# wingolab-org/pecaller

Measured on AMD Instinct MI355X. Metric: M reads mapped/sec (whole node), 2x150bp PE synthetic hg38, higher is better.
Workload: dtype f64

## Files before the change

### include/pemap_hip.h

```cpp
#ifndef PEMAP_HIP_H
#define PEMAP_HIP_H
#include <stdint.h>
#include <stddef.h>

#ifdef __cplusplus
extern "C" {
#endif

#define PEMAP_MAX_HITS   200
#define PEMAP_MIN_READ   16
#define PEMAP_MAX_READ   278

enum
{
  PEMAP_UNIQUE_MATE = 0, PEMAP_UNIQUE_SLIP = 1, PEMAP_UNIQUE_SINGLE = 2, PEMAP_UNIQUE_MIS = 3, PEMAP_NON_MATE = 4,
  PEMAP_NON_MIS = 5, PEMAP_FRAG_MIS = 6, PEMAP_NON_NO = 7, PEMAP_NEITHER_MAP = 8
};

typedef struct pemap_dev pemap_dev;

typedef void (*pemap_ins_cb) (void *user, uint32_t pos, const char *seq, int len);

const char *pemap_dev_last_error (const pemap_dev * dev);

// ... 50 lines not shown
int pemap_dev_staged_reads (pemap_dev * dev, char *reads1, int *len1, char *reads2, int *len2, int stride);
int pemap_dev_staged_info (pemap_dev * dev, int *n, int *stride, int *paired);
int pemap_dev_free (pemap_dev * dev, void *d_ptr);

typedef struct
{
  int32_t n, got[2], end[2], bad_len[2];
  uint64_t consumed[2];
} pemap_fastq_result;
int pemap_dev_stage_fastq (pemap_dev * dev, const char *text1, uint64_t bytes1, int state1, const char *text2, uint64_t bytes2, int state2,
                           int trim_start, int trim_end, int max_records, int stride, pemap_fastq_result * res);
int pemap_dev_submit_fastq (pemap_dev * dev, const char *text1, uint64_t bytes1, int state1, const char *text2, uint64_t bytes2, int state2,
                            int trim_start, int trim_end, int max_records, int stride, uint32_t * m1, uint32_t * m2, int *mapping_type,
                            pemap_fastq_result * res, uint64_t * ticket);

int pemap_dev_fetch_pileup (pemap_dev * dev, uint16_t * counts, pemap_ins_cb cb, void *user);
int pemap_dev_fetch_records (pemap_dev * dev, uint64_t first, uint64_t count, void *out, uint64_t out_capacity,
                             uint64_t * n_records);
int pemap_dev_reset_pileup (pemap_dev * dev);
int pemap_dev_absorb (pemap_dev * dst, pemap_dev * src);

int pemap_dev_summary (pemap_dev * dev, long *out13);

int pemap_dev_run_stats (pemap_dev * dev, uint64_t * stats17, float *times_ms8);

int pemap_dev_debug_hits (pemap_dev * dev, int *n_hits, uint32_t * spot, uint8_t * orient, uint32_t * win_start,
                          int *win_len, double *score, int *start_k, int *start_i);

typedef struct pecall_dev pecall_dev;
int pecall_dev_create (pecall_dev ** out, int device_id);
void pecall_dev_destroy (pecall_dev * dev);
const char *pecall_dev_last_error (const pecall_dev * dev);
int pecall_dev_site_like (pecall_dev * dev, const uint16_t * reads, const double *alpha_mean, int n_sites, int indiv,
                          int max_gen, int min_depth, double norm, double *like, int8_t * best, double *margin);
int pecall_dev_stage (pecall_dev * dev, const uint16_t * reads, const double *alpha_mean, int n_sites, int indiv);
int pecall_dev_run (pecall_dev * dev, int n_sites, int indiv, int max_gen, int min_depth, double norm, int sync);
int pecall_dev_collect (pecall_dev * dev, int n_sites, int indiv, double *like, int8_t * best, double *margin);

int pecall_dev_call_sites (pecall_dev * dev, const uint16_t * reads, const uint8_t * ref_base, const uint8_t * chrom_type, long n_sites,
                           int indiv, int haploid, double threshold, double theta, int8_t * call, double *posterior,
                           int8_t * site_type, int32_t * allele_count, int8_t * n_pass, int32_t * denovo);
int pecall_dev_call_sites_sparse (pecall_dev * dev, const uint16_t * reads, const uint8_t * ref_base, const uint8_t * chrom_type, long n_sites,
                                  int indiv, int haploid, double threshold, double theta, int8_t * call, uint32_t * post_site,
                                  double *post_rows, uint64_t post_cap, uint64_t * n_post, int8_t * site_type, int32_t * allele_count,
                                  int8_t * n_pass, int32_t * denovo);
int pecall_dev_pin_host (pecall_dev * dev, const void *host_ptr, uint64_t n_bytes);
int pecall_dev_unpin_host (pecall_dev * dev, const void *host_ptr);
// ... 39 lines not shown
```

### pecaller_amd/csrc/pemap_capi.hip

```cpp
#include <stdio.h>
#include <stdlib.h>
#include <string.h>
#include <stdarg.h>
#include <unistd.h>
#include <cstring>
#include <memory>
#include <mutex>
#include <thread>
#include <type_traits>
#include <vector>
#include "../../include/pemap_hip.h"
#include "pemap_kernels.hip.h"
#include "pemap_aux.hip.h"
#include "pemap_fastq.hip.h"
#include <rocprim/rocprim.hpp>

static char g_create_err[512] = "";
struct PmChunkCtr;

#define PM_RING 3
struct PmRingSlot
{
  bool active = false;
  unsigned long long seq = 0;
// ... 41 lines not shown
{
  char *base;
  size_t bytes;
  int users;
};
static std::mutex g_pin_mu;
static std::vector < PmPinned > g_pinned;


struct PmKnobs
{
  int big_blocks_per_cu, sw_waves_per_cu;
  int replicas;
  int gapless;
  double dir_budget_gb;
  int lookup_waves ;
  int lookup_prio, vote_prio, sw_prio;
  int vote_waves;
  int walk_blocks_per_cu, pile_blocks_per_cu;
  int pipeline;
  int chunk_pairs;
  int gapless_blocks_per_cu;
  int band, band_waves_per_cu;
  int first_tier;
  int tier2_waves;
  int absorb_staged;
  size_t absorb_chunk;
};

static int env_int (const char *name, int dflt)
{
  const char *e = getenv (name);
  return (e && *e) ? atoi (e) : dflt;
}

static void read_knobs (PmKnobs & k)
{
  k.big_blocks_per_cu = env_int ("PEMAP_BIG_BLOCKS_PER_CU", 8);
  k.sw_waves_per_cu = env_int ("PEMAP_SW_WAVES_PER_CU", 16);
  if (k.big_blocks_per_cu < 1) k.big_blocks_per_cu = 1;
  if (k.sw_waves_per_cu < 1) k.sw_waves_per_cu = 1;
  k.replicas = getenv ("PEMAP_REPLICAS") ? (env_int ("PEMAP_REPLICAS", 1) ? 1 : 0) : -1;
  k.gapless = env_int ("PEMAP_GAPLESS", 3);
  { const char *e = getenv ("PEMAP_DIR_BUDGET_GB"); k.dir_budget_gb = e ? atof (e) : 40.0; if (k.dir_budget_gb < 0.25) k.dir_budget_gb = 0.25; }
  k.lookup_waves = env_int ("PEMAP_LOOKUP_WAVES", -1);
  k.lookup_prio = env_int ("PEMAP_LOOKUP_PRIO", 0);
  k.tier2_waves = env_int ("PEMAP_TIER2_WAVES", 3);
  if (k.tier2_waves < 1) k.tier2_waves = 1;
  k.first_tier = env_int ("PEMAP_FIRST_TIER", 1);
  k.vote_prio = env_int ("PEMAP_VOTE_PRIO", 0);
  k.sw_prio = env_int ("PEMAP_SW_PRIO", 0);
  k.vote_waves = env_int ("PEMAP_VOTE_WAVES", 1024);
  if (k.vote_waves < 1) k.vote_waves = 1;
  k.walk_blocks_per_cu = env_int ("PEMAP_WALK_BLOCKS_PER_CU", 4);
  k.pile_blocks_per_cu = env_int ("PEMAP_PILE_BLOCKS_PER_CU", 4);
  if (k.walk_blocks_per_cu < 1) k.walk_blocks_per_cu = 1;
  if (k.pile_blocks_per_cu < 1) k.pile_blocks_per_cu = 1;
  k.pipeline = env_int ("PEMAP_PIPELINE", 1);
  k.chunk_pairs = env_int ("PEMAP_CHUNK_PAIRS", 262144);
  k.band = env_int ("PEMAP_BAND", 1);
  k.gapless_blocks_per_cu = env_int ("PEMAP_GAPLESS_BLOCKS_PER_CU", -1);
  if (k.gapless_blocks_per_cu == 0) k.gapless_blocks_per_cu = 1;
  k.band_waves_per_cu = env_int ("PEMAP_BAND_WAVES_PER_CU", 16);
  if (k.band_waves_per_cu < 1) k.band_waves_per_cu = 1;
  k.absorb_staged = env_int ("PEMAP_ABSORB_STAGED", 0) ? 1 : 0;
  const int kib = env_int ("PEMAP_ABSORB_CHUNK", 262144);
  k.absorb_chunk = kib > 0 ? ((size_t) kib * 1024) & ~(size_t) 255 : 0;
  if (k.absorb_chunk < 256) k.absorb_chunk = 256;
}

struct PmFastqMate
{
  uint8_t *d_text = nullptr;
  size_t text_cap = 0;
  unsigned *d_tile_cnt = nullptr;
  size_t tile_cap = 0;
  unsigned *d_line_start = nullptr;
  size_t line_cap = 0;
  PfqTileSum *d_sums = nullptr;
  uint2 *d_tile_in = nullptr;
  size_t ltile_cap = 0;
  unsigned *d_rec_off = nullptr, *d_rec_next = nullptr;
  int *d_rec_len = nullptr;
// ... 449 lines not shown
      HIPCHK (d, hipDeviceSynchronize ());
      return build_replicas (d);
    }
  return 0;
}

extern "C" int pemap_dev_lookup_replicas (pemap_dev * d, int *n_replicas, uint64_t * record_bytes)
{
  *n_replicas = d->n_rep;
  if (record_bytes)
    *record_bytes = d->n_rep ? d->multi_units * 16ull : 0ull;
  return 0;
}

extern "C" int pemap_dev_seed_launch (pemap_dev * d, int *asked, int *resident, int *launched, int *lds_bytes)
{
  *asked = d->seed_launch[0];
  *resident = d->seed_launch[1];
  *launched = d->seed_launch[2];
  *lds_bytes = d->seed_launch[3];
  return 0;
}

extern "C" int pemap_dev_index_commit (pemap_dev * d)
{
  if (!d->d_pos_index)
    return fail (d, "index_commit: no index arrays allocated");
  HIPCHK (d, hipSetDevice (d->device));
  HIPCHK (d, hipDeviceSynchronize ());
  TRY (build_replicas (d));
  d->index_ready = true;
  return 0;
}

extern "C" int pemap_dev_load_index (pemap_dev * d, const uint32_t * pos_index, const uint32_t * mers, uint64_t n_mers,
                                     const char *genome, uint64_t genome_size, const uint32_t * contig_starts, int n_contigs,
                                     int idepth)
{
  TRY (pemap_dev_index_alloc (d, n_mers, genome_size, n_contigs, idepth));
  HIPCHK (d, hipMemcpy (d->d_pos_index, pos_index, POS_INDEX_N * sizeof (uint32_t), hipMemcpyHostToDevice));
  HIPCHK (d, hipMemcpy (d->d_mers, mers, n_mers * sizeof (uint32_t), hipMemcpyHostToDevice));
  HIPCHK (d, hipMemcpy (d->d_genome, genome, genome_size, hipMemcpyHostToDevice));
  HIPCHK (d, hipMemcpy (d->d_contig_starts, contig_starts, ((size_t) n_contigs + 1) * sizeof (uint32_t), hipMemcpyHostToDevice));
  return pemap_dev_index_commit (d);
}

// ... 275 lines not shown
{
  int lanes, w;
  pick_geom (d, L, &lanes, &w);
  return (L + 21 + lanes + 15) & ~15;
}

static size_t slab_dwords_for (const pemap_dev * d, int L)
{
  int lanes, W;
  pick_geom (d, L, &lanes, &W);
  return (size_t) lanes * (size_t) tstride_for (d, L) * (size_t) ((W * 4 + 31) / 32);
}

static size_t dir_budget_bytes (const pemap_dev * d)
{
  return (size_t) (d->kn.dir_budget_gb * 1073741824.0);
}

#define PM_TASK_QUARTERS 4
struct PmTaskList
{
  uint32_t *all, *dp, *band, *c3;
  unsigned *n_all, *n_dp, *n_band, *n_c3, *dp_next, *band_next;
};

static size_t task_quarter_words (int n_ends, bool multi)
{
  return (size_t) n_ends * (multi ? PM_MAX_HITS : 1);
}

static PmTaskList task_list (const pemap_dev * d, const PmChunkSet & S, PmCounters * ctr, bool multi)
{
  uint32_t *const t = multi ? S.tasks_m : S.tasks_s;
  const size_t q = task_quarter_words (d->cap_ends, multi);
  const bool rule = pm_gapless_on (d);
  PmTaskList l;
  l.all = t;
  l.n_all = multi ? &ctr->n_tasks_m : &ctr->n_tasks_s;
  l.dp = rule ? t + q : l.all;
  l.n_dp = !rule ? l.n_all : multi ? &ctr->n_tasks_mdp : &ctr->n_tasks_dp;
  l.band = rule && d->kn.band ? t + 2 * q : nullptr;
  l.c3 = rule && pm_gapless_max_x (d) >= 3 ? t + 3 * q : nullptr;
  l.n_band = &ctr->n_band[multi];
  l.n_c3 = &ctr->n_c3[multi];
  l.dp_next = &ctr->sw_next[multi];
  l.band_next = &ctr->band_next[multi];
  return l;
}

static int alloc_hits (pemap_dev * d, PmHits & h, int n_ends)
{
  size_t nh = (size_t) n_ends * PM_MAX_HITS;
  TRY (dev_alloc (d, &h.n_hits, (size_t) n_ends));
  TRY (dev_alloc (d, &h.slot, (size_t) n_ends));
  TRY (dev_alloc (d, &h.spot, nh));
  TRY (dev_alloc (d, &h.gpos, nh));
  TRY (dev_alloc (d, &h.nn, nh));
  TRY (dev_alloc (d, &h.orient, nh));
  TRY (dev_alloc (d, &h.score, nh));
  TRY (dev_alloc (d, &h.sti, nh));
  TRY (dev_alloc (d, &h.stk, nh));
  return 0;
}

static int ensure_work (pemap_dev * d, int n_ends)
// ... 296 lines not shown
    HIPCHK (d, hipStreamWaitEvent (s.seed, *copy_ev, 0));
  if (g >= PM_SETS)
    HIPCHK (d, hipStreamWaitEvent (s.seed, S.ev_lists_free, 0));
  if (pm_fused (d))
    {
      if (g >= PM_SETS && s.ahead)
        HIPCHK (d, hipStreamWaitEvent (s.seed, S.ev_walk_done, 0));
      launch_lookup (d, c, S, cc, ev, s.seed);
      launch_rest (d, c, S, cc, s.seed);
      if (!s.emit_on_alu)
        launch_emit (d, c, S, cc, ev, s.seed);
    }
  else
    launch_lookup (d, c, S, cc, ev, s.seed);
  HIPCHK (d, hipEventRecord (S.ev_lists_ready, s.seed));
  return 0;
}

template < bool C3 > static void launch_gapless (pemap_dev * d, bool short_rows, int ggrid, const RunCtx & c, const PmChunkSet & S, const uint32_t * tasks,
                                                 const unsigned *n_tasks, const PmTaskList & l, int max_x, uint32_t * tasks_c3, unsigned *n_tasks_c3)
{
  if (short_rows)
    hipLaunchKernelGGL (HIP_KERNEL_NAME (pm_gapless_kernel < C3, true >), dim3 (ggrid), dim3 (PM_GL_BLOCK), 0, d->stream, c.ix, c.b, c.prm, S.hits, tasks, n_tasks,
                        l.dp, l.n_dp, max_x, l.band, l.n_band, tasks_c3, n_tasks_c3);
  else
    hipLaunchKernelGGL (HIP_KERNEL_NAME (pm_gapless_kernel < C3, false >), dim3 (ggrid), dim3 (PM_GL_BLOCK), 0, d->stream, c.ix, c.b, c.prm, S.hits, tasks, n_tasks,
                        l.dp, l.n_dp, max_x, l.band, l.n_band, tasks_c3, n_tasks_c3);
}

template < int W, int LPA, bool DIRS > static auto launch_cascade (pemap_dev * d, const RunCtx & c, const PmChunkSet & S, PmCounters * ctr, const PmTaskList & l)
{
  const int n_ends = c.b.n_ends, max_x = pm_gapless_max_x (d);
  int ggrid = d->n_cus * 16, bgrid = d->n_cus * d->kn.band_waves_per_cu;
  if (DIRS)
    {
      const int gbp = d->kn.gapless_blocks_per_cu > 0 ? d->kn.gapless_blocks_per_cu : (seg_template (c.L) <= 10 ? 24 : 4);
      ggrid = (n_ends + PM_GL_PER_BLOCK - 1) / PM_GL_PER_BLOCK;
      if (ggrid > d->n_cus * gbp)
        ggrid = d->n_cus * gbp;
      if (bgrid > (n_ends + 15) / 16)
        bgrid = (n_ends + 15) / 16;
    }
  const bool short_rows = seg_template (c.L) <= 10;
  if (pm_gapless_on (d))
    launch_gapless < false > (d, short_rows, ggrid, c, S, l.all, l.n_all, l, max_x, l.c3, l.n_c3);
  if (l.c3)
    launch_gapless < true > (d, short_rows, ggrid, c, S, l.c3, l.n_c3, l, max_x, (uint32_t *) nullptr, (unsigned *) nullptr);
  if (l.band)
    hipLaunchKernelGGL (HIP_KERNEL_NAME (pm_band_kernel < DIRS >), dim3 (bgrid), dim3 (64), 0, d->stream, c.ix, c.b, c.prm, S.hits, l.band, l.n_band, ctr,
                        S.dirbuf, slab_dwords_for (d, c.L), l.band_next);
  hipLaunchKernelGGL (HIP_KERNEL_NAME (pm_sw_kernel < W, LPA, DIRS >), dim3 (d->sw_grid), dim3 (64), 0, d->stream, c.ix, c.b, c.prm, S.hits, l.dp, l.n_dp, ctr,
                      S.dirbuf, S.dirbuf + c.dump_off, c.tstride, c.L, d->kn.sw_prio, l.dp_next);
}

template < int W, int LPA > static void launch_chunk (pemap_dev * d, const PmSchedule & s, const RunCtx & c, uint32_t * m1, uint32_t * m2, int *mt,
                                             PmChunkSet & S, PmChunkCtr * cc, hipEvent_t * ev)
{
  const PmHits & H = S.hits;
  uint32_t *wins = S.wins, *dirbuf = S.dirbuf;
  PmCounters *ctr = &cc->c;
  if (!pm_fused (d))
    {
      launch_vote (d, c, S, cc, ev, d->stream);
      launch_rest (d, c, S, cc, d->stream);
      launch_emit (d, c, S, cc, ev, d->stream);
    }
  else if (s.emit_on_alu)
    launch_emit (d, c, S, cc, ev, d->stream);
  launch_cascade < W, LPA, true > (d, c, S, ctr, task_list (d, S, ctr, false));
  hipEventRecord (ev[PM_EV_SW_SINGLE_END], d->stream);
// ... 40 lines not shown
            fprintf (stderr, "[pm_s4_probe]");
            for (int i = 0; i < 16; i++)
              fprintf (stderr, " %s %.1f%%", nm[i], 100.0 * (double) pr[i] / (double) tot);
            fprintf (stderr, " | total %.3f G wave-cycles | segments %llu, dropped for a too-many bucket %llu, of them by the k-mer's own bucket %llu\n", (double) tot / 1e9, pr[16], pr[17], pr[18]);
            fprintf (stderr, "[pm_s4_probe] ends decoded %llu; passed over: the list's room %llu, positions next to candidates %llu\n", pr[20], pr[21], pr[23]);
          }
        (void) hipMemcpyToSymbol (HIP_SYMBOL (pm_s4_probe), z, sizeof z);
      }
  }
#endif
  std::vector < PmChunkCtr > hc (nch);
  HIPCHK (d, hipMemcpy (hc.data (), d->d_chunk_ctr, sizeof (PmChunkCtr) * nch, hipMemcpyDeviceToHost));
  HIPCHK (d, hipMemcpy (&d->last_cur, d->d_cur, sizeof (PmInsCursor), hipMemcpyDeviceToHost));
  PmCounters & t = d->last_ctr;
  for (int k = 0; k < nch; k++)
    {
      const PmCounters & c = hc[k].c;
      t.n_tasks_s += c.n_tasks_s;
      t.n_tasks_m += c.n_tasks_m;
      t.n_tasks_dp += pm_gapless_on (d) ? c.n_tasks_dp : c.n_tasks_s;
      t.n_tasks_mdp += pm_gapless_on (d) ? c.n_tasks_mdp : c.n_tasks_m;
      t.n_band[0] += c.n_band[0];
      t.n_band[1] += c.n_band[1];
      t.cells_band += c.cells_band;
      t.n_slots += c.n_slots;
      t.n_redo += c.n_redo;
      t.n_wins += c.n_wins;
      t.n_walks += c.n_walks;
      t.positions += c.positions + hc[k].positions;
      t.cells_score += c.cells_score;
      t.cells_dirs += c.cells_dirs;
      t.pile_incs += c.pile_incs;
      t.n_ins += c.n_ins;
      d->last_big += hc[k].n_big;
      d->last_big2 += hc[k].n_big2;
      hipEvent_t *ev = &d->evs[(size_t) k * PM_NEV];
      float ms = 0.f;
      for (const auto & iv : pm_intervals)
        if (hipEventElapsedTime (&ms, ev[iv.from], ev[iv.to]) == hipSuccess)
          {
            d->last_ms[iv.slot] += ms;
            d->last_ms[PM_T_SEED] += iv.seed_too ? ms : 0.f;
          }
    }
  if (d->last_cur.ins_overflow)
    return fail (d, "insertion log overflow (%u bytes): lower PEMAP_CHUNK_PAIRS or map smaller slices", d->ins_cap);
// ... 619 lines not shown
extern "C" int pemap_dev_run_stats (pemap_dev * d, uint64_t * s, float *t)
{
  TRY (pemap_dev_sync (d));
  const PmCounters & c = d->last_ctr;
  if (s)
    {
      s[0] = d->run_ends;
      s[1] = c.positions;
      s[2] = (uint64_t) c.n_tasks_s + c.n_tasks_m;
      s[3] = (uint64_t) c.n_tasks_dp + c.n_band[0] + c.n_redo;
      s[4] = c.cells_score;
      s[5] = c.cells_dirs;
      s[6] = c.pile_incs;
      s[7] = c.n_ins;
      s[8] = c.n_wins;
      s[9] = c.n_redo;
      s[10] = d->last_big;
      s[11] = (uint64_t) d->run_chunks;
      s[12] = ((uint64_t) c.n_tasks_s - c.n_tasks_dp - c.n_band[0]) + ((uint64_t) c.n_tasks_m - c.n_tasks_mdp - c.n_band[1]);
      s[13] = (uint64_t) c.n_band[0] + c.n_band[1];
      s[14] = c.cells_band;
      s[15] = d->last_big2;
      s[16] = c.n_walks;
    }
  if (t)
    memcpy (t, d->last_ms, sizeof (d->last_ms));
  return 0;
}

extern "C" int pemap_dev_debug_hits (pemap_dev * d, int *n_hits, uint32_t * spot, uint8_t * orient, uint32_t * win_start,
                                     int *win_len, double *score, int *start_k, int *start_i)
{
  HIPCHK (d, hipSetDevice (d->device));
  HIPCHK (d, hipStreamSynchronize (d->stream));
  const int n_ends = d->paired ? 2 * d->run_n : d->run_n;
  const size_t nh = (size_t) n_ends * PM_MAX_HITS;
  const PmHits & H = d->set[0].hits;
  if (n_hits)
    HIPCHK (d, hipMemcpy (n_hits, H.n_hits, (size_t) n_ends * sizeof (int), hipMemcpyDeviceToHost));
  if (spot)
    HIPCHK (d, hipMemcpy (spot, H.spot, nh * 4, hipMemcpyDeviceToHost));
  if (orient)
    HIPCHK (d, hipMemcpy (orient, H.orient, nh, hipMemcpyDeviceToHost));
  if (win_start)
    HIPCHK (d, hipMemcpy (win_start, H.gpos, nh * 4, hipMemcpyDeviceToHost));
  if (score)
// ... 609 lines not shown
```

### pecaller_amd/csrc/pemap_kernels.hip.h

```cpp
#pragma once
#include <hip/hip_runtime.h>
#include <stdint.h>
#include "pemap_pile_diff.h"

#define PM_MAX_HITS 200
#define PM_TOO_MANY 100
#define PM_SLOP 10
#define PM_MAX_SEG 19
#define PM_SEED_CAP 1024
#define PM_SEG_LIST_MAX 4851
#define PM_WAVES_PER_EU(W) ((W) <= 13 ? 4 : (W) <= 19 ? 3 : (W) <= 32 ? 2 : 1)
#define PM_SW_WAVES_PER_EU(W, DIRS) ((W) <= 10 ? 4 : (W) <= 13 ? 3 : (W) <= 16 ? ((DIRS) ? 3 : 2) : ((DIRS) ? 2 : 3))

struct PmIndex
{
  const uint32_t *pos_index;
  const uint32_t *mers;
  const uint8_t *genome;
  const uint32_t *contig_starts;
  uint64_t n_mers;
  uint64_t gsize;
  int n_contigs;
  int idepth;
  const uint32_t *rep;
// ... 59 lines not shown
  return (uint16_t) (p.w[(size_t) q * p.plane_words + (pos >> 1)] >> (16 * (pos & 1)));
}

struct PmCounters
{
  unsigned int n_tasks_s;
  unsigned int n_tasks_m;
  unsigned int n_slots;
  unsigned int n_redo;
  unsigned int n_wins;
  unsigned int n_tasks_dp;
  unsigned long long positions;
  unsigned long long cells_score;
  unsigned long long cells_dirs;
  unsigned long long pile_incs;
  unsigned long long n_ins;
  unsigned int sw_next[3];
  unsigned int n_tasks_mdp;
  unsigned int n_band[2];
  unsigned int band_next[2];
  unsigned int n_c3[2];
  unsigned long long cells_band;
  unsigned int n_walks;
};

struct PmInsCursor
{
  unsigned int ins_bytes;
  unsigned int ins_overflow;
};

struct PmHits
{
  int *n_hits;
  uint32_t *spot;
  uint32_t *gpos;
  int16_t *nn;
  uint8_t *orient;
  double *score;
  int16_t *sti;
  uint8_t *stk;
  int *slot;
};

struct PmBatch
{
// ... 123 lines not shown
```

### pecaller_amd/csrc/pemap_sw.hip.h

```cpp
#pragma once

#define PM_GO 2.0
#define PM_GE (1.0 / 36.0)
#define PM_NEGBIG (-1.0e30)

__device__ __forceinline__ double pm_border (int j)
{
  return -(PM_GO + (double) (j - 1) * PM_GE);
}

__device__ __forceinline__ double pm_top (int j)
{
  return (j >= 1) ? pm_border (j) : (double) j;
}

__device__ __forceinline__ double pm_max (double a, double b)
{
  return __builtin_fmax (a, b);
}

__device__ __forceinline__ bool pm_match (uint8_t r, uint8_t q, int bis)
{
  bool m = (r == q) | (q == 'N') | (q == 'n');
  m |= (r == 'N') & (q >= 'N');
// ... 341 lines not shown
{
  const uint64_t vv = v | (0x4141414141414141ull & ~(~0ull << vacated_bits));
  const uint32_t lo = (uint32_t) vv, hi = (uint32_t) (vv >> 32);
  const uint32_t clo = pm_comp4 (lo), chi = pm_comp4 (hi);
  if (pm_comp4 (clo) == lo && pm_comp4 (chi) == hi)
    return ((uint64_t) __builtin_amdgcn_perm (0u, clo, 0x00010203u) << 32) | (uint64_t) __builtin_amdgcn_perm (0u, chi, 0x00010203u);
  uint64_t w = 0;
#pragma unroll
  for (int k = 0; k < 8; k++)
    w |= (uint64_t) pm_rc_flat ((uint8_t) (v >> (8 * (7 - k)))) << (8 * k);
  return w;
}

#define PM_GAPLESS 4
#define PM_GL_QUEUE 32
#define PM_GL_QUEUE_SHORT 24

#ifndef PM_BAND_K
#define PM_BAND_K 5
#endif
#define PM_BAND_W (22 + 2 * PM_BAND_K)
#define PM_BAND_MAXX_ (PM_BAND_K >= 5 ? 6 : PM_BAND_K + 1)
static_assert (PM_BAND_K >= 2 && PM_BAND_K <= 5, "the band holds at most 32 diagonals");
#define PM_GL_BLOCK 64
#define PM_GL_PER_BLOCK (PM_GL_BLOCK / 32)
#ifndef PM_GL_WAVES_PER_EU
#define PM_GL_WAVES_PER_EU 4
#endif
#define PM_GL_SHORT_MM 160
template < bool SHORT > struct PmGlRows
{
  static constexpr int RD = SHORT ? (PM_GL_SHORT_MM + 7) / 8 * 8 : 320;
  static constexpr int WIN = SHORT ? 16 + (PM_GL_SHORT_MM + 2 * PM_SLOP + 1 + 15) / 8 * 8 : 360;
  static constexpr int QUEUE = SHORT ? PM_GL_QUEUE_SHORT : PM_GL_QUEUE;
};
static_assert (PmGlRows < true >::RD == 160 && PmGlRows < true >::WIN == 208, "short rows as derived above");
static_assert (PM_GL_PER_BLOCK * (PmGlRows < true >::RD + PmGlRows < true >::WIN) + 3 * 4 * PmGlRows < true >::QUEUE <= 1024, "the short form's LDS budget");
template < bool C3, bool SHORT > __global__ __launch_bounds__ (PM_GL_BLOCK, PM_GL_WAVES_PER_EU) void pm_gapless_kernel (PmIndex ix, PmBatch b, PmParams prm, PmHits h, const uint32_t * tasks,
                                                          const unsigned *n_tasks_p, uint32_t * tasks_dp, unsigned *n_tasks_dp, int max_x,
                                                          uint32_t * tasks_band, unsigned *n_tasks_band, uint32_t * tasks_c3, unsigned *n_tasks_c3)
{
  using Rows = PmGlRows < SHORT >;
  constexpr int QN = Rows::QUEUE;
  __shared__ __align__ (8) uint8_t rd[PM_GL_PER_BLOCK][Rows::RD];
  __shared__ __align__ (8) uint8_t win[PM_GL_PER_BLOCK][Rows::WIN];
  __shared__ uint32_t q_band[PM_GL_BLOCK / 64][QN], q_dp[PM_GL_BLOCK / 64][QN];
  __shared__ uint32_t q_c3[PM_GL_BLOCK / 64][C3 ? 1 : QN];
  const int wv = threadIdx.x >> 6;
  int n_qb = 0, n_qd = 0, n_q3 = 0;
  auto flush_queue = [&] (const uint32_t * q, int &n, uint32_t * dst, unsigned *counter)
  {
    if (n == 0)
      return;
    const unsigned base = (unsigned) __builtin_amdgcn_readfirstlane ((int) ((threadIdx.x & 63) == 0 ? atomicAdd (counter, (unsigned) n) : 0u));
    __builtin_amdgcn_fence (__ATOMIC_SEQ_CST, "wavefront");
    __builtin_amdgcn_wave_barrier ();
    if ((int) (threadIdx.x & 63) < n)
      dst[base + (threadIdx.x & 63)] = q[threadIdx.x & 63];
    n = 0;
    __builtin_amdgcn_fence (__ATOMIC_SEQ_CST, "wavefront");
    __builtin_amdgcn_wave_barrier ();
  };
  const int lane = threadIdx.x & 63, l = lane & 31, half = lane & 32;
  const int slot = threadIdx.x >> 5;
  const unsigned n_tasks = *n_tasks_p;
  const int bis = prm.bisulfite;
  const double miss = __hiloint2double ((int) 0xBFD55555u, (int) 0x55555555u);
  const unsigned stride = gridDim.x * (unsigned) PM_GL_PER_BLOCK;
  struct Meta
  {
    size_t o;
    int mm, nn, orient;
// ... 304 lines not shown
      double sc = 0.0;
      if ((cmask >> l) & 1u)
        {
          if (mism >= 1)
            {
              sc = (double) m1 + miss;
              int at = m1;
              for (int k = 1; k < mism; k++)
                {
                  const int nxt = k == 1 ? m2 : mlast;
                  sc = pm_add_ones (sc, nxt - at - 1);
                  sc = sc + miss;
                  at = nxt;
                }
              sc = pm_add_ones (sc, mm - at - 1);
            }
          else
            sc = (double) mm;
        }
      {
        int xmin = mism;
        for (int s = 16; s; s >>= 1)
          xmin = min (xmin, __shfl_xor (xmin, s));
        const bool to_c3 = !C3 && valid && cmask == 0u && l == 0 && tasks_c3 && xmin == 3 && ndiag == 2 * PM_SLOP + 2;
        const bool open = valid && cmask == 0u && l == 0 && !to_c3;
        const bool to_band = open && tasks_band && xmin <= PM_BAND_MAXX_, to_dp = open && !to_band;
        const unsigned long long mb = __ballot (to_band), md = __ballot (to_dp);
        if (to_band)
          q_band[wv][n_qb + (int) __popcll (mb & ((1ull << lane) - 1ull))] = (uint32_t) o;
        if (to_dp)
          q_dp[wv][n_qd + (int) __popcll (md & ((1ull << lane) - 1ull))] = (uint32_t) o;
        n_qb += (int) __popcll (mb);
        n_qd += (int) __popcll (md);
        if (n_qb > QN - 2)
          flush_queue (q_band[wv], n_qb, tasks_band, n_tasks_band);
        if (n_qd > QN - 2)
          flush_queue (q_dp[wv], n_qd, tasks_dp, n_tasks_dp);
        if (!C3)
          {
            const unsigned long long m3 = __ballot (to_c3);
            if (to_c3)
              q_c3[wv][n_q3 + (int) __popcll (m3 & ((1ull << lane) - 1ull))] = (uint32_t) o;
            n_q3 += (int) __popcll (m3);
            if (n_q3 > QN - 2)
              flush_queue (q_c3[wv], n_q3, tasks_c3, n_tasks_c3);
          }
      }
      if (valid)
        {
// ... 8 lines not shown
                  m &= m - 1u;
                  const double s = __shfl (sc, half + dl);
                  if (bd < 0 || s > best)
                    {
                      best = s;
                      bd = dl;
                    }
                }
              if (l == 0)
                {
                  h.score[o] = best;
                  h.stk[o] = (uint8_t) PM_GAPLESS;
                  h.sti[o] = (int16_t) (bd + mm);
                }
            }
        }
      __builtin_amdgcn_fence (__ATOMIC_SEQ_CST, "wavefront");
      __builtin_amdgcn_wave_barrier ();
    }
  flush_queue (q_band[wv], n_qb, tasks_band, n_tasks_band);
  flush_queue (q_dp[wv], n_qd, tasks_dp, n_tasks_dp);
  if (!C3)
    flush_queue (q_c3[wv], n_q3, tasks_c3, n_tasks_c3);
}

__device__ __forceinline__ int pm_wave_max (int v)
{
  for (int o = 32; o > 0; o >>= 1)
    v = max (v, __shfl_xor (v, o));
  return v;
}

template < int W, int PM_LPA, bool DIRS > __global__ __launch_bounds__ (64, PM_SW_WAVES_PER_EU (W, DIRS)) void pm_sw_kernel (PmIndex ix, PmBatch b, PmParams prm, PmHits h,
                                                                                              const uint32_t * tasks,
                                                                                              const unsigned *n_tasks_p, PmCounters * ctr,
                                                                                              uint32_t * dirbuf, uint32_t * dump_slab, int tstride,
                                                                                              int mm_fill, int prio, unsigned *next_task)
{
  constexpr int TPW = 64 / PM_LPA;
  __shared__ uint32_t stage[DIRS ? 64 * PM_STAGE_OF (PmSwGeom < W >::DW) * PmSwGeom < W >::DW : 4];
  __shared__ uint32_t *slab_of_group[TPW + 1];
  pm_set_prio (prio);
  const int lane = threadIdx.x;
  const int q = lane / PM_LPA;
  const unsigned n_tasks = *n_tasks_p;
  if (blockIdx.x * (unsigned) TPW >= n_tasks)
// ... 564 lines not shown
```

### pecaller_amd/pemap.py

```python
import ctypes as C
import os
import numpy as np

HERE = os.path.dirname(os.path.abspath(__file__))
LIB_PATH = os.environ.get("PEMAP_LIB") or os.path.join(HERE, "libpemap_hip.so")
MAX_HITS = 200
MIN_READ = 16
MAX_READ = 278
CLASS_NAMES = ["UNIQUE_MATE", "UNIQUE_SLIP", "UNIQUE_SINGLE", "UNIQUE_MIS", "NON_MATE", "NON_MIS", "FRAG_MIS", "NON_NO",
               "NEITHER_MAP"]

SYMBOLS = [
    "pemap_dev_last_error", "pemap_dev_create", "pemap_dev_destroy", "pemap_dev_load_index", "pemap_dev_build_index",
    "pemap_dev_build_index_resident", "pemap_dev_index_alloc", "pemap_dev_index_commit", "pemap_dev_set_lookup_replicas",
    "pemap_dev_lookup_replicas", "pemap_dev_buffer",
    "pemap_dev_index_info", "pemap_dev_read_buffer", "pemap_dev_set_params", "pemap_dev_map_batch",
    "pemap_dev_submit_batch", "pemap_dev_wait_batch", "pemap_dev_pin_host", "pemap_dev_unpin_host",
    "pemap_dev_stage_reads", "pemap_dev_run", "pemap_dev_run_slice", "pemap_dev_collect", "pemap_dev_sync",
    "pemap_dev_synth_genome", "pemap_dev_synth_reads", "pemap_dev_synth_reads_indel", "pemap_dev_staged_reads", "pemap_dev_staged_info",
    "pemap_dev_free", "pemap_dev_fetch_pileup", "pemap_dev_fetch_records", "pemap_dev_reset_pileup", "pemap_dev_summary",
    "pemap_dev_run_stats", "pemap_dev_debug_hits", "pemap_dev_index_share", "pemap_dev_absorb",
    "pecall_dev_create", "pecall_dev_destroy", "pecall_dev_last_error", "pecall_dev_site_like", "pecall_dev_stage",
    "pecall_dev_run", "pecall_dev_collect", "pecall_dev_call_sites", "pecall_dev_call_sites_sparse", "pecall_dev_set_pedigree",
    "pecall_dev_sites_stage", "pecall_dev_sites_run", "pecall_dev_sites_stats", "pecall_dev_sites_collect", "pecall_dev_pin_host", "pecall_dev_unpin_host",
    "pecall_dev_sites_stage_records", "pecall_dev_sites_gather", "pecall_dev_sites_merge_ms", "pecall_dev_call_records",
    "pecall_dev_sites_stage_records_guided", "pecall_dev_call_records_guided",
    "pecall_dev_sites_base_text",
    "pemap_dev_stage_fastq", "pemap_dev_submit_fastq", "pemap_dev_seed_launch",
]

FASTQ_TILE = 4096
FASTQ_LINE_TILE = 1024
FASTQ_TOP = 1024
FASTQ_MAX_TEXT = 1 << 30


class FastqResult(C.Structure):
    _fields_ = [("n", C.c_int32), ("got", C.c_int32 * 2), ("end", C.c_int32 * 2), ("bad_len", C.c_int32 * 2), ("consumed", C.c_uint64 * 2)]

    def as_dict(self):
        return dict(n=self.n, got=list(self.got), end=list(self.end), bad_len=list(self.bad_len), consumed=list(self.consumed))


PILE_DT = np.dtype([("pos", "<u4"), ("c", "<u2", (6,))])
# ... 32 lines not shown
        L.pemap_dev_read_buffer.argtypes = [vp, i, u64, vp, u64]
        L.pemap_dev_set_params.argtypes = [vp, i, i, i, dbl, i]
        L.pemap_dev_map_batch.argtypes = [vp, vp, vp, vp, vp, i, i, vp, vp, vp]
        L.pemap_dev_submit_batch.argtypes = [vp, vp, vp, vp, vp, i, i, vp, vp, vp, C.POINTER(u64)]
        L.pemap_dev_wait_batch.argtypes = [vp, u64]
        L.pemap_dev_pin_host.argtypes = [vp, vp, u64]
        L.pemap_dev_unpin_host.argtypes = [vp, vp]
        L.pemap_dev_stage_reads.argtypes = [vp, vp, vp, vp, vp, i, i]
        L.pemap_dev_run.argtypes = [vp, i]
        L.pemap_dev_run_slice.argtypes = [vp, i, i, i]
        L.pemap_dev_collect.argtypes = [vp, vp, vp, vp]
        L.pemap_dev_sync.argtypes = [vp]
        L.pemap_dev_synth_genome.argtypes = [vp, u64, u64, i, dbl, C.POINTER(vp), vp]
        L.pemap_dev_synth_reads.argtypes = [vp, u64, i, i, i, dbl, dbl, u64]
        L.pemap_dev_synth_reads_indel.argtypes = [vp, u64, i, i, i, dbl, dbl, u64]
        L.pemap_dev_staged_reads.argtypes = [vp, vp, vp, vp, vp, i]
        L.pemap_dev_staged_info.argtypes = [vp, C.POINTER(i), C.POINTER(i), C.POINTER(i)]
        L.pemap_dev_free.argtypes = [vp, vp]
        L.pemap_dev_fetch_pileup.argtypes = [vp, vp, vp, vp]
        L.pemap_dev_fetch_records.argtypes = [vp, u64, u64, vp, u64, C.POINTER(u64)]
        L.pemap_dev_reset_pileup.argtypes = [vp]
        L.pemap_dev_summary.argtypes = [vp, vp]
        L.pemap_dev_run_stats.argtypes = [vp, vp, vp]
        L.pemap_dev_debug_hits.argtypes = [vp, vp, vp, vp, vp, vp, vp, vp, vp]
        L.pemap_dev_index_share.argtypes = [vp, vp]
        L.pemap_dev_absorb.argtypes = [vp, vp]
        fq = [vp, C.c_char_p, u64, i, C.c_char_p, u64, i, i, i, i, i]
        L.pemap_dev_stage_fastq.argtypes = fq + [C.POINTER(FastqResult)]
        L.pemap_dev_submit_fastq.argtypes = fq + [vp, vp, vp, C.POINTER(FastqResult), C.POINTER(u64)]
        _lib = L
    return _lib


INS_CB = C.CFUNCTYPE(None, C.c_void_p, C.c_uint32, C.c_char_p, C.c_int)


def _p(a):
    return None if a is None else a.ctypes.data


class PemapDev:

    def __init__(self, device_id=0):
        self.L = load_library()
        h = C.c_void_p()
        if self.L.pemap_dev_create(C.byref(h), device_id):
# ... 35 lines not shown
        self._ck(self.L.pemap_dev_index_alloc(self.h, n_mers, genome_size, n_contigs, idepth))
        self.gsize = genome_size

    def index_commit(self):
        self._ck(self.L.pemap_dev_index_commit(self.h))

    def index_share(self, src):
        self._ck(self.L.pemap_dev_index_share(self.h, src.h))
        self.gsize = src.gsize

    def set_lookup_replicas(self, n):
        self._ck(self.L.pemap_dev_set_lookup_replicas(self.h, int(n)))

    def lookup_replicas(self):
        n = C.c_int(0)
        b = C.c_uint64(0)
        self._ck(self.L.pemap_dev_lookup_replicas(self.h, C.byref(n), C.byref(b)))
        return n.value, b.value

    def seed_launch(self):
        v = [C.c_int(0) for _ in range(4)]
        self._ck(self.L.pemap_dev_seed_launch(self.h, *[C.byref(x) for x in v]))
        return dict(zip(("asked", "resident", "launched", "lds_bytes"), (x.value for x in v)))

    def index_info(self):
        a, b, c, d = C.c_uint64(), C.c_uint64(), C.c_int(), C.c_int()
        self._ck(self.L.pemap_dev_index_info(self.h, C.byref(a), C.byref(b), C.byref(c), C.byref(d)))
        return a.value, b.value, c.value, d.value

    def buffer(self, which):
        p, n = C.c_void_p(), C.c_uint64()
        self._ck(self.L.pemap_dev_buffer(self.h, which, C.byref(p), C.byref(n)))
        return p.value, n.value

    def read_buffer(self, which, dtype, offset_bytes=0, n_bytes=None):
        _, nb = self.buffer(which)
        if n_bytes is None:
            n_bytes = nb - offset_bytes
        out = np.empty(n_bytes // np.dtype(dtype).itemsize, dtype=dtype)
        self._ck(self.L.pemap_dev_read_buffer(self.h, which, offset_bytes, _p(out), n_bytes))
        return out

    def set_params(self, paired=True, min_dist=0, max_dist=500, min_align=0.85, bisulfite=False):
        self.paired = bool(paired)
        self._ck(self.L.pemap_dev_set_params(self.h, int(paired), min_dist, max_dist, min_align, int(bisulfite)))

# ... 120 lines not shown
        return counts, sorted(ins)

    def fetch_records(self, first=0, count=None):
        count = self.gsize - first if count is None else count
        n = C.c_uint64()
        self._ck(self.L.pemap_dev_fetch_records(self.h, first, count, None, 0, C.byref(n)))
        out = np.zeros(n.value, PILE_DT)
        if n.value:
            self._ck(self.L.pemap_dev_fetch_records(self.h, first, count, _p(out), n.value, C.byref(n)))
        return out

    def reset_pileup(self):
        self._ck(self.L.pemap_dev_reset_pileup(self.h))

    def absorb(self, src):
        self._ck(self.L.pemap_dev_absorb(self.h, src.h))

    def summary(self):
        out = np.zeros(13, np.int64)
        self._ck(self.L.pemap_dev_summary(self.h, _p(out)))
        return out

    def run_stats(self):
        s = np.zeros(17, np.uint64)
        t = np.zeros(8, np.float32)
        self._ck(self.L.pemap_dev_run_stats(self.h, _p(s), _p(t)))
        keys = ["ends", "positions", "sw_score", "sw_dirs", "cells_score", "cells_dirs", "pile_incs", "n_ins", "walks", "redo", "big_ends", "chunks", "gapless", "banded", "cells_band", "mono_ends", "walked"]
        tk = ["seed", "sw_single", "sw_multi", "select", "sw_redo", "walk", "lookup", "vote"]
        return dict(zip(keys, (int(x) for x in s))), dict(zip(tk, (float(x) for x in t)))

    def debug_hits(self, n_ends):
        nh = np.zeros(n_ends, np.int32)
        spot = np.zeros((n_ends, MAX_HITS), np.uint32)
        orient = np.zeros((n_ends, MAX_HITS), np.uint8)
        ws = np.zeros((n_ends, MAX_HITS), np.uint32)
        wl = np.zeros((n_ends, MAX_HITS), np.int32)
        sc = np.zeros((n_ends, MAX_HITS), np.float64)
        sk = np.zeros((n_ends, MAX_HITS), np.int32)
        si = np.zeros((n_ends, MAX_HITS), np.int32)
        self._ck(self.L.pemap_dev_debug_hits(self.h, _p(nh), _p(spot), _p(orient), _p(ws), _p(wl), _p(sc), _p(sk), _p(si)))
        return dict(n_hits=nh, spot=spot, orient=orient, win_start=ws, win_len=wl, score=sc, start_k=sk, start_i=si)
```

Measured before the change: 118.3.

## Gate high-mismatch gapless candidates into the banded kernel instead of full DP

Ends that fail the gapless mismatch threshold and span two or more diagonals are now sent to the C3 gapless pass. There, a wave-level bound built from the first and last mismatch positions decides whether a small-band indel alignment could reach the best score. Ends that pass this gate go to the banded kernel rather than full Smith-Waterman DP, to cut expensive DP work. This adds a routing pass, shuffles and an atomic counter. By default it is disabled for small batches relative to the SW grid.

```diff
diff --git a/include/pemap_hip.h b/include/pemap_hip.h
--- a/include/pemap_hip.h
+++ b/include/pemap_hip.h
@@ -96,7 +96,9 @@
 
 int pemap_dev_summary (pemap_dev * dev, long *out13);
 
-int pemap_dev_run_stats (pemap_dev * dev, uint64_t * stats17, float *times_ms8);
+int pemap_dev_sw_grid (pemap_dev * dev);
+
+int pemap_dev_run_stats (pemap_dev * dev, uint64_t * stats18, float *times_ms8);
 
 int pemap_dev_debug_hits (pemap_dev * dev, int *n_hits, uint32_t * spot, uint8_t * orient, uint32_t * win_start,
                           int *win_len, double *score, int *start_k, int *start_i);
diff --git a/pecaller_amd/csrc/pemap_capi.hip b/pecaller_amd/csrc/pemap_capi.hip
--- a/pecaller_amd/csrc/pemap_capi.hip
+++ b/pecaller_amd/csrc/pemap_capi.hip
@@ -87,6 +87,7 @@
   int chunk_pairs;
   int gapless_blocks_per_cu;
   int band, band_waves_per_cu;
+  int band_gate;
   int first_tier;
   int tier2_waves;
   int absorb_staged;
@@ -124,6 +125,7 @@
   k.pipeline = env_int ("PEMAP_PIPELINE", 1);
   k.chunk_pairs = env_int ("PEMAP_CHUNK_PAIRS", 262144);
   k.band = env_int ("PEMAP_BAND", 1);
+  k.band_gate = getenv ("PEMAP_BAND_GATE") ? (env_int ("PEMAP_BAND_GATE", 1) ? 1 : 0) : -1;
   k.gapless_blocks_per_cu = env_int ("PEMAP_GAPLESS_BLOCKS_PER_CU", -1);
   if (k.gapless_blocks_per_cu == 0) k.gapless_blocks_per_cu = 1;
   k.band_waves_per_cu = env_int ("PEMAP_BAND_WAVES_PER_CU", 16);
@@ -619,6 +621,11 @@
   return 0;
 }
 
+extern "C" int pemap_dev_sw_grid (pemap_dev * d)
+{
+  return d->sw_grid;
+}
+
 extern "C" int pemap_dev_index_commit (pemap_dev * d)
 {
   if (!d->d_pos_index)
@@ -940,6 +947,7 @@
 {
   uint32_t *all, *dp, *band, *c3;
   unsigned *n_all, *n_dp, *n_band, *n_c3, *dp_next, *band_next;
+  unsigned *n_gate;
 };
 
 static size_t task_quarter_words (int n_ends, bool multi)
@@ -958,7 +966,8 @@
   l.dp = rule ? t + q : l.all;
   l.n_dp = !rule ? l.n_all : multi ? &ctr->n_tasks_mdp : &ctr->n_tasks_dp;
   l.band = rule && d->kn.band ? t + 2 * q : nullptr;
-  l.c3 = rule && pm_gapless_max_x (d) >= 3 ? t + 3 * q : nullptr;
+  l.n_gate = l.band && d->kn.band_gate ? &ctr->n_gate[multi] : nullptr;
+  l.c3 = rule && (pm_gapless_max_x (d) >= 3 || l.n_gate) ? t + 3 * q : nullptr;
   l.n_band = &ctr->n_band[multi];
   l.n_c3 = &ctr->n_c3[multi];
   l.dp_next = &ctr->sw_next[multi];
@@ -1301,15 +1310,18 @@
 {
   if (short_rows)
     hipLaunchKernelGGL (HIP_KERNEL_NAME (pm_gapless_kernel < C3, true >), dim3 (ggrid), dim3 (PM_GL_BLOCK), 0, d->stream, c.ix, c.b, c.prm, S.hits, tasks, n_tasks,
-                        l.dp, l.n_dp, max_x, l.band, l.n_band, tasks_c3, n_tasks_c3);
+                        l.dp, l.n_dp, max_x, l.band, l.n_band, tasks_c3, n_tasks_c3, l.n_gate);
   else
     hipLaunchKernelGGL (HIP_KERNEL_NAME (pm_gapless_kernel < C3, false >), dim3 (ggrid), dim3 (PM_GL_BLOCK), 0, d->stream, c.ix, c.b, c.prm, S.hits, tasks, n_tasks,
-                        l.dp, l.n_dp, max_x, l.band, l.n_band, tasks_c3, n_tasks_c3);
+                        l.dp, l.n_dp, max_x, l.band, l.n_band, tasks_c3, n_tasks_c3, l.n_gate);
 }
 
 template < int W, int LPA, bool DIRS > static auto launch_cascade (pemap_dev * d, const RunCtx & c, const PmChunkSet & S, PmCounters * ctr, const PmTaskList & l)
 {
   const int n_ends = c.b.n_ends, max_x = pm_gapless_max_x (d);
+  PmTaskList lg = l;
+  if (d->kn.band_gate < 0 && (long) n_ends <= (long) d->sw_grid * (64 / LPA))
+    lg.n_gate = nullptr;
   int ggrid = d->n_cus * 16, bgrid = d->n_cus * d->kn.band_waves_per_cu;
   if (DIRS)
     {
@@ -1322,9 +1334,9 @@
     }
   const bool short_rows = seg_template (c.L) <= 10;
   if (pm_gapless_on (d))
-    launch_gapless < false > (d, short_rows, ggrid, c, S, l.all, l.n_all, l, max_x, l.c3, l.n_c3);
+    launch_gapless < false > (d, short_rows, ggrid, c, S, l.all, l.n_all, lg, max_x, l.c3, l.n_c3);
   if (l.c3)
-    launch_gapless < true > (d, short_rows, ggrid, c, S, l.c3, l.n_c3, l, max_x, (uint32_t *) nullptr, (unsigned *) nullptr);
+    launch_gapless < true > (d, short_rows, ggrid, c, S, l.c3, l.n_c3, lg, max_x, (uint32_t *) nullptr, (unsigned *) nullptr);
   if (l.band)
     hipLaunchKernelGGL (HIP_KERNEL_NAME (pm_band_kernel < DIRS >), dim3 (bgrid), dim3 (64), 0, d->stream, c.ix, c.b, c.prm, S.hits, l.band, l.n_band, ctr,
                         S.dirbuf, slab_dwords_for (d, c.L), l.band_next);
@@ -1411,6 +1423,8 @@
       t.n_tasks_mdp += pm_gapless_on (d) ? c.n_tasks_mdp : c.n_tasks_m;
       t.n_band[0] += c.n_band[0];
       t.n_band[1] += c.n_band[1];
+      t.n_gate[0] += c.n_gate[0];
+      t.n_gate[1] += c.n_gate[1];
       t.cells_band += c.cells_band;
       t.n_slots += c.n_slots;
       t.n_redo += c.n_redo;
@@ -2076,6 +2090,7 @@
       s[14] = c.cells_band;
       s[15] = d->last_big2;
       s[16] = c.n_walks;
+      s[17] = (uint64_t) c.n_gate[0] + c.n_gate[1];
     }
   if (t)
     memcpy (t, d->last_ms, sizeof (d->last_ms));
diff --git a/pecaller_amd/csrc/pemap_kernels.hip.h b/pecaller_amd/csrc/pemap_kernels.hip.h
--- a/pecaller_amd/csrc/pemap_kernels.hip.h
+++ b/pecaller_amd/csrc/pemap_kernels.hip.h
@@ -105,6 +105,7 @@
   unsigned int n_c3[2];
   unsigned long long cells_band;
   unsigned int n_walks;
+  unsigned int n_gate[2];
 };
 
 struct PmInsCursor
diff --git a/pecaller_amd/csrc/pemap_sw.hip.h b/pecaller_amd/csrc/pemap_sw.hip.h
--- a/pecaller_amd/csrc/pemap_sw.hip.h
+++ b/pecaller_amd/csrc/pemap_sw.hip.h
@@ -387,6 +387,9 @@
 #define PM_BAND_W (22 + 2 * PM_BAND_K)
 #define PM_BAND_MAXX_ (PM_BAND_K >= 5 ? 6 : PM_BAND_K + 1)
 static_assert (PM_BAND_K >= 2 && PM_BAND_K <= 5, "the band holds at most 32 diagonals");
+#define PM_GATE_Y 2
+#define PM_GATE_LOSS36 (PM_BAND_K >= 5 ? 288 : 0)
+static_assert (PM_GATE_Y == 2, "pm_gapless_kernel keeps p0..p2 and s0..s2 in named registers");
 #define PM_GL_BLOCK 64
 #define PM_GL_PER_BLOCK (PM_GL_BLOCK / 32)
 #ifndef PM_GL_WAVES_PER_EU
@@ -403,7 +406,8 @@
 static_assert (PM_GL_PER_BLOCK * (PmGlRows < true >::RD + PmGlRows < true >::WIN) + 3 * 4 * PmGlRows < true >::QUEUE <= 1024, "the short form's LDS budget");
 template < bool C3, bool SHORT > __global__ __launch_bounds__ (PM_GL_BLOCK, PM_GL_WAVES_PER_EU) void pm_gapless_kernel (PmIndex ix, PmBatch b, PmParams prm, PmHits h, const uint32_t * tasks,
                                                           const unsigned *n_tasks_p, uint32_t * tasks_dp, unsigned *n_tasks_dp, int max_x,
-                                                          uint32_t * tasks_band, unsigned *n_tasks_band, uint32_t * tasks_c3, unsigned *n_tasks_c3)
+                                                          uint32_t * tasks_band, unsigned *n_tasks_band, uint32_t * tasks_c3, unsigned *n_tasks_c3,
+                                                          unsigned *n_gate)
 {
   using Rows = PmGlRows < SHORT >;
   constexpr int QN = Rows::QUEUE;
@@ -413,6 +417,7 @@
   __shared__ uint32_t q_c3[PM_GL_BLOCK / 64][C3 ? 1 : QN];
   const int wv = threadIdx.x >> 6;
   int n_qb = 0, n_qd = 0, n_q3 = 0;
+  int n_gated = 0;
   auto flush_queue = [&] (const uint32_t * q, int &n, uint32_t * dst, unsigned *counter)
   {
     if (n == 0)
@@ -763,9 +768,74 @@
         int xmin = mism;
         for (int s = 16; s; s >>= 1)
           xmin = min (xmin, __shfl_xor (xmin, s));
-        const bool to_c3 = !C3 && valid && cmask == 0u && l == 0 && tasks_c3 && xmin == 3 && ndiag == 2 * PM_SLOP + 2;
+        const bool two_diag = n_gate && tasks_band && xmin > PM_BAND_MAXX_ && ndiag >= 2;
+        bool gated = false;
+        if (C3 && two_diag)
+          {
+            int p0 = mm, p1 = mm, p2 = mm, s0 = mm, s1 = mm, s2 = mm;
+            if (mine)
+              {
+                int nf = 0;
+                for (int c = 0; c < nch && nf < PM_GATE_Y + 1; c++)
+                  for (unsigned mk = piece_mask (l, c); mk != 0u && nf < PM_GATE_Y + 1; mk &= mk - 1u, nf++)
+                    {
+                      const int at = 8 * c + __ffs ((int) mk) - 1;
+                      if (nf == 0)
+                        p0 = at;
+                      else if (nf == 1)
+                        p1 = at;
+                      else
+                        p2 = at;
+                    }
+                nf = 0;
+                for (int c = nch - 1; c >= 0 && nf < PM_GATE_Y + 1; c--)
+                  for (unsigned mk = piece_mask (l, c); mk != 0u && nf < PM_GATE_Y + 1; nf++)
+                    {
+                      const int bit = 31 - __clz ((int) mk);
+                      mk &= ~(1u << bit);
+                      const int len = mm - 1 - (8 * c + bit);
+                      if (nf == 0)
+                        s0 = len;
+                      else if (nf == 1)
+                        s1 = len;
+                      else
+                        s2 = len;
+                    }
+              }
+            else
+              p0 = p1 = p2 = s0 = s1 = s2 = 0;
+            const int P[PM_GATE_Y + 1] = { p0, p1, p2 };
+            constexpr bool del_ok = 72 + 2 * PM_SLOP + 48 * 2 * PM_GATE_Y <= PM_GATE_LOSS36;
+            int pmax = p2;
+            for (int s = 1; s < 32; s <<= 1)
+              {
+                const int v = __shfl_up (pmax, s);
+                if (l >= s)
+                  pmax = max (pmax, v);
+              }
+            int pbefore = __shfl_up (pmax, 1);
+            if (l == 0)
+              pbefore = 0;
+            bool adm = del_ok && mine && pbefore + s2 >= mm;
+#pragma unroll
+            for (int bb = 1; bb <= PM_BAND_K; bb++)
+              {
+                const int src = half + (l >= bb ? l - bb : l);
+                const int T[PM_GATE_Y + 1] = { __shfl (s0, src), __shfl (s1, src), __shfl (s2, src) };
+#pragma unroll
+                for (int i = 0; i <= PM_GATE_Y; i++)
+#pragma unroll
+                  for (int j = 0; j <= PM_GATE_Y; j++)
+                    if (36 * bb + 72 + (bb - 1) + 48 * (i + j) <= PM_GATE_LOSS36)
+                      adm |= mine && l >= bb && P[i] + T[j] >= mm - bb;
+              }
+            gated = (unsigned) (__ballot (adm) >> half) != 0u;
+          }
+        if (C3)
+          n_gated += (int) __popcll (__ballot (gated && l == 0));
+        const bool to_c3 = !C3 && valid && cmask == 0u && l == 0 && tasks_c3 && ((xmin == 3 && ndiag == 2 * PM_SLOP + 2) || two_diag);
         const bool open = valid && cmask == 0u && l == 0 && !to_c3;
-        const bool to_band = open && tasks_band && xmin <= PM_BAND_MAXX_, to_dp = open && !to_band;
+        const bool to_band = open && tasks_band && (xmin <= PM_BAND_MAXX_ || gated), to_dp = open && !to_band;
         const unsigned long long mb = __ballot (to_band), md = __ballot (to_dp);
         if (to_band)
           q_band[wv][n_qb + (int) __popcll (mb & ((1ull << lane) - 1ull))] = (uint32_t) o;
@@ -820,6 +890,8 @@
   flush_queue (q_dp[wv], n_qd, tasks_dp, n_tasks_dp);
   if (!C3)
     flush_queue (q_c3[wv], n_q3, tasks_c3, n_tasks_c3);
+  if (C3 && n_gated > 0 && lane == 0)
+    atomicAdd (n_gate, (unsigned) n_gated);
 }
 
 __device__ __forceinline__ int pm_wave_max (int v)
diff --git a/pecaller_amd/pemap.py b/pecaller_amd/pemap.py
--- a/pecaller_amd/pemap.py
+++ b/pecaller_amd/pemap.py
@@ -19,7 +19,7 @@
     "pemap_dev_stage_reads", "pemap_dev_run", "pemap_dev_run_slice", "pemap_dev_collect", "pemap_dev_sync",
     "pemap_dev_synth_genome", "pemap_dev_synth_reads", "pemap_dev_synth_reads_indel", "pemap_dev_staged_reads", "pemap_dev_staged_info",
     "pemap_dev_free", "pemap_dev_fetch_pileup", "pemap_dev_fetch_records", "pemap_dev_reset_pileup", "pemap_dev_summary",
-    "pemap_dev_run_stats", "pemap_dev_debug_hits", "pemap_dev_index_share", "pemap_dev_absorb",
+    "pemap_dev_run_stats", "pemap_dev_sw_grid", "pemap_dev_debug_hits", "pemap_dev_index_share", "pemap_dev_absorb",
     "pecall_dev_create", "pecall_dev_destroy", "pecall_dev_last_error", "pecall_dev_site_like", "pecall_dev_stage",
     "pecall_dev_run", "pecall_dev_collect", "pecall_dev_call_sites", "pecall_dev_call_sites_sparse", "pecall_dev_set_pedigree",
     "pecall_dev_sites_stage", "pecall_dev_sites_run", "pecall_dev_sites_stats", "pecall_dev_sites_collect", "pecall_dev_pin_host", "pecall_dev_unpin_host",
@@ -98,6 +98,8 @@
         L.pemap_dev_reset_pileup.argtypes = [vp]
         L.pemap_dev_summary.argtypes = [vp, vp]
         L.pemap_dev_run_stats.argtypes = [vp, vp, vp]
+        if hasattr(L, "pemap_dev_sw_grid"):
+            L.pemap_dev_sw_grid.argtypes = [vp]
         L.pemap_dev_debug_hits.argtypes = [vp, vp, vp, vp, vp, vp, vp, vp, vp]
         L.pemap_dev_index_share.argtypes = [vp, vp]
         L.pemap_dev_absorb.argtypes = [vp, vp]
@@ -179,6 +181,9 @@
         v = [C.c_int(0) for _ in range(4)]
         self._ck(self.L.pemap_dev_seed_launch(self.h, *[C.byref(x) for x in v]))
         return dict(zip(("asked", "resident", "launched", "lds_bytes"), (x.value for x in v)))
+
+    def sw_grid(self):
+        return int(self.L.pemap_dev_sw_grid(self.h))
 
     def index_info(self):
         a, b, c, d = C.c_uint64(), C.c_uint64(), C.c_int(), C.c_int()
@@ -345,10 +350,10 @@
         return out
 
     def run_stats(self):
-        s = np.zeros(17, np.uint64)
+        s = np.zeros(18, np.uint64)
         t = np.zeros(8, np.float32)
         self._ck(self.L.pemap_dev_run_stats(self.h, _p(s), _p(t)))
-        keys = ["ends", "positions", "sw_score", "sw_dirs", "cells_score", "cells_dirs", "pile_incs", "n_ins", "walks", "redo", "big_ends", "chunks", "gapless", "banded", "cells_band", "mono_ends", "walked"]
+        keys = ["ends", "positions", "sw_score", "sw_dirs", "cells_score", "cells_dirs", "pile_incs", "n_ins", "walks", "redo", "big_ends", "chunks", "gapless", "banded", "cells_band", "mono_ends", "walked", "gated"]
         tk = ["seed", "sw_single", "sw_multi", "select", "sw_redo", "walk", "lookup", "vote"]
         return dict(zip(keys, (int(x) for x in s))), dict(zip(tk, (float(x) for x in t)))
 
```

After: 123.0, median of 6. +4.0%, better.
